# iden3/snarkjs

Hardware: AMD Instinct MI355X
Metric: groth16_proofs_per_sec (higher is better)
Workload: dtype u32; 1 GPU; BN254 Groth16 prove, 2^20 constraints, synthetic zkey/wtns (BASELINE configs[1]), B density 1.0 (every section dense, SURVEY 8d recipe), uniform witness; key + witness resident in HBM; curve=bn128, log_n=20, n_vars=1048571, n_coef=2097203, witness=uniform, coef_dist=flat, parallelism=replica x1 (one proof stream per GPU, 2 proof(s) in flight)

## Files before the change

### snarkjs_amd/csrc/msm29.cuh

```cuda
#pragma once
#include "field29.cuh"
#include "msm.cuh"

namespace zkmi {

#if defined(ZK29_SHADOW)
}
#include <map>
namespace zkmi {
namespace b29 {
struct Parked { double bv, bl, bt; };
inline std::map<const void*, Parked>& parked() { static std::map<const void*, Parked> m; return m; }
}
#endif
template <class C> struct Aff29 { Fp29<C> x, y; };
template <class C> struct XYZZ29 { Fp29<C> X, Y, ZZ, ZZZ; };

template <class C> ZK_HD void dbl_affine29(XYZZ29<C>& r, const Aff29<C>& q) {
    Fp29<C> U = add29(q.y, q.y); norm29(U);
    const Fp29<C> V = mul29(U, U), W = mul29(U, V), S = mul29(q.x, V), xx = mul29(q.x, q.x);
    Fp29<C> M = add29(add29(xx, xx), xx); norm29(M);
    Fp29<C> X3 = sub29<C, 2>(sub29<C, 2>(mul29(M, M), S), S); norm29(X3);
    const Fp29<C> T = sub29<C, 6>(S, X3);
    Fp29<C> Y3 = sub29<C, 2>(mul29(M, T), mul29(W, q.y)); norm29(Y3);
    r.X = X3; r.Y = Y3; r.ZZ = V; r.ZZZ = W;
}
template <class C> ZK_HD void madd29(XYZZ29<C>& acc, bool& inf, const Aff29<C>& q) {
    if (inf) { acc.X = q.x; acc.Y = q.y; acc.ZZ = one29<C>(); acc.ZZZ = one29<C>(); inf = false; return; }
    const Fp29<C> U2 = mul29(q.x, acc.ZZ), S2 = mul29(q.y, acc.ZZZ);
    Fp29<C> P = sub29<C, 8>(U2, acc.X); norm29(P);
    Fp29<C> R = sub29<C, 4>(S2, acc.Y); norm29(R);
    if (is_zero29(P)) {
        if (is_zero29(R)) dbl_affine29(acc, q); else inf = true;
        return;
    }
    const Fp29<C> PP = sqr29(P);
    const Fp29<C> PPP = mul29(P, PP), Q = mul29(acc.X, PP);
    Fp29<C> X3 = sub29<C, 2>(sub29<C, 2>(sub29<C, 2>(sqr29(R), PPP), Q), Q); norm29(X3);
    Fp29<C> T = sub29<C, 8>(Q, X3); norm29(T);
    const Fp29<C> Y3 = mul29_2(R, T, sub29<C, 4>(zero29<C>(), acc.Y), PPP);
    acc.ZZ = mul29(acc.ZZ, PP); acc.ZZZ = mul29(acc.ZZZ, PPP);
    acc.X = X3; acc.Y = Y3;
}
template <class C, bool KEEP29 = false> ZK_HD void store_xyzz29(uint32_t* dst, const XYZZ29<C>& a, bool inf) {
    constexpr int N = C::N;
    if (inf) {
#pragma unroll
        for (int i = 0; i < N; i++) reinterpret_cast<uint4*>(dst)[i] = make_uint4(0, 0, 0, 0);
        return;
    }
    store_r256<C, KEEP29>(dst, a.X); store_r256<C, KEEP29>(dst + N, a.Y); store_r256<C, KEEP29>(dst + 2 * N, a.ZZ); store_r256<C, KEEP29>(dst + 3 * N, a.ZZZ);
}
template <class C> ZK_HD bool load_xyzz29(XYZZ29<C>& a, const uint32_t* src) {
    constexpr int N = C::N;
    const uint4* q = reinterpret_cast<const uint4*>(src + 2 * N);
    uint32_t nz = 0;
#pragma unroll
    for (int i = 0; i < N / 4; i++) { const uint4 z = q[i]; nz |= z.x | z.y | z.z | z.w; }
    if (!nz) return false;
    a.X = load29_packed<C>(src); a.Y = load29_packed<C>(src + N); a.ZZ = load29_packed<C>(src + 2 * N); a.ZZZ = load29_packed<C>(src + 3 * N);
    return true;
}
template <class C> ZK_HD void dbl_xyzz29(XYZZ29<C>& r) {
    Fp29<C> U = add29(r.Y, r.Y); norm29(U);
    const Fp29<C> V = sqr29(U), W = mul29(U, V), S = mul29(r.X, V), xx = sqr29(r.X);
    Fp29<C> M = add29(add29(xx, xx), xx); norm29(M);
    Fp29<C> X3 = sub29<C, 2>(sub29<C, 2>(sqr29(M), S), S); norm29(X3);
    Fp29<C> T = sub29<C, 6>(S, X3); norm29(T);
    const Fp29<C> Y3 = mul29_2(M, T, sub29<C, 2>(zero29<C>(), W), r.Y);
    r.ZZ = mul29(V, r.ZZ); r.ZZZ = mul29(W, r.ZZZ);
    r.X = X3; r.Y = Y3;
}
template <class C, class Ld> ZK_HD void padd29_ld(XYZZ29<C>& acc, bool& inf, Ld ld) {
    if (inf) { acc.X = ld(0); acc.Y = ld(1); acc.ZZ = ld(2); acc.ZZZ = ld(3); inf = false; return; }
    const Fp29<C> U1 = mul29(acc.X, ld(2)), U2 = mul29(ld(0), acc.ZZ);
    Fp29<C> P = sub29<C, 2>(U2, U1); norm29(P);
    const Fp29<C> S1 = mul29(acc.Y, ld(3)), S2 = mul29(ld(1), acc.ZZZ);
    Fp29<C> R = sub29<C, 2>(S2, S1); norm29(R);
    if (is_zero29(P)) {
        if (is_zero29(R)) dbl_xyzz29(acc); else inf = true;
        return;
    }
    const Fp29<C> PP = sqr29(P);
    const Fp29<C> PPP = mul29(P, PP), Q = mul29(U1, PP);
    Fp29<C> X3 = sub29<C, 2>(sub29<C, 2>(sub29<C, 2>(sqr29(R), PPP), Q), Q); norm29(X3);
    Fp29<C> T = sub29<C, 8>(Q, X3); norm29(T);
    const Fp29<C> Y3 = mul29_2(R, T, sub29<C, 2>(zero29<C>(), S1), PPP);
    acc.ZZ = mul29(mul29(acc.ZZ, ld(2)), PP); acc.ZZZ = mul29(mul29(acc.ZZZ, ld(3)), PPP);
    acc.X = X3; acc.Y = Y3;
}
template <class C> ZK_HD void padd29(XYZZ29<C>& acc, bool& inf, const XYZZ29<C>& p) {
    padd29_ld(acc, inf, [&](int k) -> Fp29<C> { return k == 0 ? p.X : (k == 1 ? p.Y : (k == 2 ? p.ZZ : p.ZZZ)); });
}
template <class C> ZK_HD bool xyzz29_words_inf(const uint32_t* src) {
    const uint4* q = reinterpret_cast<const uint4*>(src + 2 * C::N);
    uint32_t nz = 0;
#pragma unroll
    for (int i = 0; i < C::N / 4; i++) { const uint4 z = q[i]; nz |= z.x | z.y | z.z | z.w; }
    return nz == 0;
}


template <class C> ZK_HD bool xyzz29_words_inf_g2(const uint32_t* src) {
    const uint4* q = reinterpret_cast<const uint4*>(src + 4 * C::N);
    uint32_t nz = 0;
#pragma unroll
    for (int i = 0; i < C::N / 2; i++) { const uint4 z = q[i]; nz |= z.x | z.y | z.z | z.w; }
    return nz == 0;
}

template <class C> __global__ void __launch_bounds__(256) k_table_to_r29(uint32_t* __restrict__ table, size_t n_elems) {
    const size_t i = (size_t)blockIdx.x * blockDim.x + threadIdx.x;
    if (i >= n_elems) return;
    Fp<C> v = fp_load<C>(table + i * C::N);
#pragma unroll
    for (int k = 0; k < r29_shift<C>(); k++) v = fp_dbl(v);
    fp_store<C>(table + i * C::N, v);
}

struct ListReader {
    const uint4* sorted4;
    uint32_t a, a_end, at = 0xffffffffu;
    uint4 buf;
    ZK_DEV ListReader(const uint32_t* sorted, uint32_t first, uint32_t last) : sorted4(reinterpret_cast<const uint4*>(sorted)), a(first), a_end(last), buf(make_uint4(0, 0, 0, 0)) {}
    ZK_DEV bool more() const { return a < a_end; }
    ZK_DEV uint32_t next() {
        const uint32_t grp = a >> 2, sel = a & 3u;
        if (grp != at) { buf = sorted4[grp]; at = grp; }
        a++;
        return sel == 0 ? buf.x : (sel == 1 ? buf.y : (sel == 2 ? buf.z : buf.w));
    }
};
#ifndef ZK_SPEC_GATHER
#define ZK_SPEC_GATHER 1
#endif
#ifndef ZK_SPEC_GATHER_G2
#define ZK_SPEC_GATHER_G2(C) (ZK_SPEC_GATHER && Lim29<C>::NL > 9)
#endif
struct SpecEntry { uint32_t e, m, s; };
ZK_DEV bool spec_dead(const SpecEntry& x) { return x.s >= 32u || ((x.m >> x.s) & 1u); }
template <class C> ZK_DEV Fp29<C> unpack29_v(const uint4* v) {
    uint32_t w[C::N];
#pragma unroll
    for (int i = 0; i < C::N / 4; i++) { w[4 * i] = v[i].x; w[4 * i + 1] = v[i].y; w[4 * i + 2] = v[i].z; w[4 * i + 3] = v[i].w; }
    return unpack29<C>(w);
}

template <class C, bool MERGE> __global__ void __launch_bounds__(256, 2)
k_msm_accum29(const uint32_t* __restrict__ bases, const uint32_t* __restrict__ infmask, MsmShape sh, uint32_t skip, uint32_t cap, const uint32_t* __restrict__ counts,
              const uint32_t* __restrict__ starts, const uint32_t* __restrict__ sorted, const uint32_t* __restrict__ lane_g, const uint32_t* __restrict__ lane_sub,
              const uint32_t* __restrict__ meta, uint32_t* __restrict__ buckets, uint32_t* __restrict__ lane_partials, const uint32_t* __restrict__ prev_counts, int bucket_r29) {
    constexpr int N = C::N, PW = 4 * N, AV = N / 2;
    const uint32_t lane = blockIdx.x * blockDim.x + threadIdx.x;
    if (lane >= meta[0]) return;
    const uint32_t g = lane_g[lane];
    const uint32_t cnt = counts[g];
    const uint32_t j = msm_key_lanes_log(msm_key(cnt, cap), cap);
    uint32_t lo = 0, hi = cnt;
    if (j) {
        const uint32_t chunk = (cnt + (1u << j) - 1) >> j;
        lo = min(cnt, lane_sub[lane] * chunk);
        hi = min(cnt, lo + chunk);
    }
    XYZZ29<C> acc;
    bool inf = true;
    if (MERGE) {
        if (prev_counts[g] && (!j || lane_sub[lane] == 0)) {
            const uint32_t* b = buckets + (size_t)g * PW;
            if (bucket_r29) inf = !load_xyzz29(acc, b);
            else {
                uint32_t nz = 0;
#pragma unroll
                for (int i = 0; i < N / 4; i++) { const uint4 z = reinterpret_cast<const uint4*>(b + 2 * N)[i]; nz |= z.x | z.y | z.z | z.w; }
                if (nz) { acc.X = from_r256<C>(b); acc.Y = from_r256<C>(b + N); acc.ZZ = from_r256<C>(b + 2 * N); acc.ZZZ = from_r256<C>(b + 3 * N); inf = false; }
            }
        }
    }
    const uint32_t s0 = starts[g];
    ListReader list(sorted, s0 + lo, s0 + hi);
    struct Raw { uint4 v[AV]; };
    auto fetch = [&](uint32_t& e_out, Raw& r_out) -> bool {
        while (list.more()) {
            const uint32_t e = list.next();
            uint32_t idx = e & 0x7fffffffu;
            if (idx < skip) continue;
            idx -= skip;
            if ((infmask[idx >> 5] >> (idx & 31)) & 1u) continue;
            const uint4* p = reinterpret_cast<const uint4*>(bases + (size_t)idx * (2 * N));
#pragma unroll
            for (int i = 0; i < AV; i++) r_out.v[i] = p[i];
            e_out = e;
            return true;
        }
        return false;
    };
#if ZK_SPEC_GATHER
    auto fetch_spec = [&](SpecEntry& x, Raw& r_out) -> bool {
        if (!list.more()) return false;
        const uint32_t e = list.next();
        uint32_t idx = e & 0x7fffffffu;
        const bool mine = idx >= skip;
        idx = mine ? idx - skip : 0u;
        x.e = e; x.s = mine ? (idx & 31u) : 32u;
        x.m = infmask[idx >> 5];
        const uint4* p = reinterpret_cast<const uint4*>(bases + (size_t)idx * (2 * N));
#pragma unroll
        for (int i = 0; i < AV; i++) r_out.v[i] = p[i];
        return true;
    };
    SpecEntry x_next{0, 0, 32};
    Raw r_next;
    bool have = fetch_spec(x_next, r_next);
    while (have) {
        SpecEntry x = x_next;
        Raw r = r_next;
        have = fetch_spec(x_next, r_next);
        while (spec_dead(x) && have) { x = x_next; r = r_next; have = fetch_spec(x_next, r_next); }
        if (spec_dead(x)) break;
        Aff29<C> q;
        q.x = unpack29_v<C>(r.v); q.y = unpack29_v<C>(r.v + AV / 2);
        if (x.e >> 31) { q.y = sub29<C, 2>(zero29<C>(), q.y); norm29(q.y); }
        madd29(acc, inf, q);
    }
#else
    uint32_t e_next = 0;
    Raw r_next;
    bool have = fetch(e_next, r_next);
    while (have) {
        const uint32_t e = e_next;
        const Raw r = r_next;
        have = fetch(e_next, r_next);
        Aff29<C> q;
        q.x = unpack29_v<C>(r.v); q.y = unpack29_v<C>(r.v + AV / 2);
        if (e >> 31) { q.y = sub29<C, 2>(zero29<C>(), q.y); norm29(q.y); }
        madd29(acc, inf, q);
    }
#endif
    if (j) store_xyzz29<C, false>(lane_partials + (size_t)lane * PW, acc, inf);
    else if (bucket_r29) store_xyzz29<C, true>(buckets + (size_t)g * PW, acc, inf);
    else store_xyzz29<C, false>(buckets + (size_t)g * PW, acc, inf);
}

template <class C> __global__ void __launch_bounds__(256, Lim29<C>::NL <= 9 ? 3 : 2)
k_msm_rowcol_wave29(MsmReduceBatch rb, uint32_t W, uint32_t nb, uint32_t rbits, uint32_t cbits, uint32_t* __restrict__ out) {
    constexpr int NL = Lim29<C>::NL, PW = 4 * C::N;
    extern __shared__ __attribute__((aligned(16))) uint32_t lds[];
    __shared__ uint32_t inf_s[256];
    const uint32_t Cn = 1u << cbits, R = 1u << rbits;
    const uint32_t t = threadIdx.x, sub = t & 63u;
    const size_t n_out = (size_t)rb.njobs * W * 2 * Cn;
    for (size_t blk = blockIdx.x; blk * 4 < n_out; blk += gridDim.x) {
        const size_t gw = blk * 4 + (t >> 6);
        const bool valid = gw < n_out;
        const uint32_t i = (uint32_t)(gw & (Cn - 1)), kind = (uint32_t)(gw >> cbits) & 1u;
        const size_t jw = gw >> (cbits + 1);
        const uint32_t w = (uint32_t)(jw % W), job = (uint32_t)(jw / W);
        XYZZ29<C> acc;
        bool inf = true;
        if (valid) {
            const uint32_t* bk = rb.buckets[job];
            const uint32_t* cn = rb.counts[job];
            const uint32_t cnt = kind ? R : Cn;
            if (!kind && i >= R) {  }
            else for (uint32_t e = sub; e < cnt; e += 64) {
                const size_t g = (size_t)w * nb + (kind ? ((size_t)e << cbits) + i : ((size_t)i << cbits) + e);
                const uint32_t* src = bk + g * PW;
                if (cn[g] && !xyzz29_words_inf<C>(src)) padd29_ld(acc, inf, [&](int k) { return load29_packed<C>(src + k * C::N); });
            }
        }
        uint32_t* mine = lds + t;
        for (uint32_t d = 1; d < 64; d <<= 1) {
            inf_s[t] = inf ? 1u : 0u;
            if (!inf) {
#pragma unroll
                for (int k = 0; k < NL; k++) { mine[k * 256] = acc.X.l[k]; mine[(NL + k) * 256] = acc.Y.l[k]; mine[(2 * NL + k) * 256] = acc.ZZ.l[k]; mine[(3 * NL + k) * 256] = acc.ZZZ.l[k]; }
            }
            __syncthreads();
            if ((t & (2 * d - 1)) == 0 && !inf_s[t + d]) {
                const uint32_t* pn = lds + t + d;
                padd29_ld(acc, inf, [&](int k) { Fp29<C> v;
#pragma unroll
                    for (int i = 0; i < NL; i++) v.l[i] = pn[(k * NL + i) * 256];
                    return v; });
            }
            __syncthreads();
        }
        if (valid && sub == 0) store_xyzz29<C, false>(out + gw * PW, acc, inf);
    }
}

template <class C> struct F2x { Fp29<C> c0, c1; };
template <class C, int K> ZK_HD Fp29<C> neg29(const Fp29<C>& a) { Fp29<C> r = sub29<C, K>(zero29<C>(), a); norm29(r); return r; }
#define ZK_F2_CALLS(C) (IsCompact<C>::value)
template <class C> __host__ __device__ ZK_NOINLINE_DEV F2x<C> f2mul_call(F2x<C> a, F2x<C> b) {
    static_assert(Lim29<C>::NL > 9, "called Fq2 product: 14-limb curve only (offset 16 p needs its headroom)");
    const Fp29<C> nb1 = neg29<C, 16>(b.c1);
    return F2x<C>{mul29_2_inl(a.c0, b.c0, a.c1, nb1), mul29_2_inl(a.c0, b.c1, a.c1, b.c0)};
}
template <class C> ZK_HD F2x<C> f2mul(const F2x<C>& a, const F2x<C>& b, const Fp29<C>& nb1) {
    if constexpr (ZK_F2_CALLS(C)) return f2mul_call<C>(a, b);
    else return F2x<C>{mul29_2(a.c0, b.c0, a.c1, nb1), mul29_2(a.c0, b.c1, a.c1, b.c0)};
}
template <class C, int KB> ZK_HD F2x<C> f2sqr(const F2x<C>& a) {
    Fp29<C> s = add29(a.c0, a.c1), d = sub29<C, KB>(a.c0, a.c1);
    norm29(d);
    Fp29<C> t = mul29(a.c0, a.c1);
    Fp29<C> c1 = add29(t, t);
    norm29(c1);
    return F2x<C>{mul29(s, d), c1};
}
template <class C, int K> ZK_HD F2x<C> f2sub(const F2x<C>& a, const F2x<C>& b) { return F2x<C>{sub29<C, K>(a.c0, b.c0), sub29<C, K>(a.c1, b.c1)}; }
template <class C> ZK_HD void f2norm(F2x<C>& a) { norm29(a.c0); norm29(a.c1); }
template <class C> ZK_HD bool f2zero(const F2x<C>& a) { return is_zero29(a.c0) && is_zero29(a.c1); }

template <class C, int T, bool PACK> struct LdsAcc29 {
    static constexpr int NL = Lim29<C>::NL, EW = PACK ? C::N : NL;
    uint32_t* base;
    ZK_HD void get1(int slot, Fp29<C>& v) const {
        if constexpr (PACK) {
            uint32_t w[C::N];
#pragma unroll
            for (int i = 0; i < C::N; i++) w[i] = base[(slot * EW + i) * T];
            v = unpack29<C>(w);
        } else {
#pragma unroll
            for (int i = 0; i < NL; i++) v.l[i] = base[(slot * EW + i) * T];
        }
#if defined(ZK29_SHADOW)
        {
            auto it = b29::parked().find(&base[(size_t)slot * EW * T]);
            b29::need(it != b29::parked().end(), "LdsAcc29: slot read before it was written", slot, 0);
            if (it != b29::parked().end()) { v.bv = it->second.bv; v.bl = it->second.bl; v.bt = it->second.bt; }
        }
#endif
    }
    ZK_HD void put1(int slot, const Fp29<C>& v) const {
#if defined(ZK29_SHADOW)
        {
            b29::need(b29::normalised(v), "LdsAcc29: a parked value is not normalised", v.bl, b29::lowmax<C>());
            b29::Parked pk; pk.bv = v.bv; pk.bl = v.bl; pk.bt = v.bt;
            b29::parked()[&base[(size_t)slot * EW * T]] = pk;
        }
#endif
        if constexpr (PACK) {
            uint32_t w[C::N];
            pack29<C>(w, v);
#pragma unroll
            for (int i = 0; i < C::N; i++) base[(slot * EW + i) * T] = w[i];
        } else {
#pragma unroll
            for (int i = 0; i < NL; i++) base[(slot * EW + i) * T] = v.l[i];
        }
    }
    ZK_HD void get(int coord, F2x<C>& v) const { get1(2 * coord, v.c0); get1(2 * coord + 1, v.c1); }
    ZK_HD void put(int coord, const F2x<C>& v) const { put1(2 * coord, v.c0); put1(2 * coord + 1, v.c1); }
};
#ifndef ZK_Y3_SPLIT
#define ZK_Y3_SPLIT(C) (Lim29<C>::NL > 9 || IsCompact<C>::value)
#endif
#ifndef ZK_G2_PREFETCH
#define ZK_G2_PREFETCH(C) true
#endif
#if defined(__HIP_DEVICE_COMPILE__)
#define ZK_SFENCE() __builtin_amdgcn_sched_barrier(0)
#else
#define ZK_SFENCE() ((void)0)
#endif
template <class C, class Acc> ZK_HD void madd29_lds(const Acc& A, bool& inf, const F2x<C>& qx, const F2x<C>& qy) {
    F2x<C> t;
    if (inf) {
        A.put(0, qx); A.put(1, qy);
        t.c0 = one29<C>(); t.c1 = zero29<C>();
        A.put(2, t); A.put(3, t);
        inf = false;
        return;
    }
    A.get(2, t);
    const F2x<C> U2 = f2mul(t, qx, neg29<C, 2>(qx.c1));
    ZK_SFENCE();
    A.get(0, t);
    F2x<C> P = f2sub<C, 9>(U2, t); f2norm(P);
    A.get(3, t);
    const F2x<C> S2 = f2mul(t, qy, neg29<C, 3>(qy.c1));
    ZK_SFENCE();
    A.get(1, t);
    F2x<C> R = f2sub<C, 4>(S2, t); f2norm(R);
    if (f2zero(P)) {
        if (f2zero(R)) {
            F2x<C> U{add29(qy.c0, qy.c0), add29(qy.c1, qy.c1)}; f2norm(U);
            const F2x<C> V = f2sqr<C, 5>(U);
            const Fp29<C> nV1 = neg29<C, 3>(V.c1);
            const F2x<C> W = f2mul(U, V, nV1), S = f2mul(qx, V, nV1);
            const F2x<C> xx = f2sqr<C, 2>(qx);
            F2x<C> M{add29(add29(xx.c0, xx.c0), xx.c0), add29(add29(xx.c1, xx.c1), xx.c1)}; f2norm(M);
            F2x<C> X3 = f2sub<C, 2>(f2sub<C, 2>(f2sqr<C, 7>(M), S), S); f2norm(X3);
            F2x<C> Tt = f2sub<C, 7>(S, X3); f2norm(Tt);
            const F2x<C> MT = f2mul(M, Tt, neg29<C, 9>(Tt.c1)), Wy = f2mul(W, qy, neg29<C, 3>(qy.c1));
            F2x<C> Y3 = f2sub<C, 2>(MT, Wy); f2norm(Y3);
            A.put(0, X3); A.put(1, Y3); A.put(2, V); A.put(3, W);
        } else inf = true;
        return;
    }
    const F2x<C> PP = f2sqr<C, 11>(P);
    ZK_SFENCE();
    const Fp29<C> nPP1 = neg29<C, 4>(PP.c1);
    const F2x<C> PPP = f2mul(P, PP, nPP1);
    ZK_SFENCE();
    const Fp29<C> nPPP1 = neg29<C, 2>(PPP.c1);
    A.get(2, t); A.put(2, f2mul(t, PP, nPP1));
    ZK_SFENCE();
    A.get(3, t); A.put(3, f2mul(t, PPP, nPPP1));
    ZK_SFENCE();
    A.get(0, t);
    const F2x<C> Q = f2mul(t, PP, nPP1);
    ZK_SFENCE();
    F2x<C> X3 = f2sub<C, 2>(f2sub<C, 2>(f2sub<C, 2>(f2sqr<C, 6>(R), PPP), Q), Q); f2norm(X3);
    A.put(0, X3);
    ZK_SFENCE();
    F2x<C> Tq = f2sub<C, 9>(Q, X3); f2norm(Tq);
    const Fp29<C> nR1 = neg29<C, 6>(R.c1);
    F2x<C> Y3;
    if constexpr (ZK_Y3_SPLIT(C)) {
        const F2x<C> TR{mul29_2(Tq.c0, R.c0, Tq.c1, nR1), mul29_2(Tq.c0, R.c1, Tq.c1, R.c0)};
        ZK_SFENCE();
        const Fp29<C> nPPP0 = neg29<C, 2>(PPP.c0);
        A.get(1, t);
        Y3.c0 = add29(TR.c0, mul29_2(t.c0, nPPP0, t.c1, PPP.c1));
        Y3.c1 = add29(TR.c1, mul29_2(t.c0, nPPP1, t.c1, nPPP0));
        f2norm(Y3);
    } else {
        const Fp29<C> nPPP0 = neg29<C, 2>(PPP.c0);
        A.get(1, t);
        Y3.c0 = mul29_4(Tq.c0, R.c0, Tq.c1, nR1, t.c0, nPPP0, t.c1, PPP.c1);
        Y3.c1 = mul29_4(Tq.c0, R.c1, Tq.c1, R.c0, t.c0, nPPP1, t.c1, nPPP0);
    }
    A.put(1, Y3);
}
template <class C, class Acc, bool KEEP29 = false> ZK_HD void store_xyzz29_lds(uint32_t* dst, const Acc& A, bool inf) {
    constexpr int N = C::N;
    if (inf) {
#pragma unroll
        for (int i = 0; i < 2 * N; i++) reinterpret_cast<uint4*>(dst)[i] = make_uint4(0, 0, 0, 0);
// ... 496 lines not shown
```

### snarkjs_amd/csrc/msm_host.hpp

```cpp
#pragma once
#include <stdlib.h>
#include <string.h>
#include <algorithm>
#include "host_field.hpp"
#include "msm.cuh"
#include "msm29.cuh"
#include <type_traits>
#include "zkmi_common.hpp"
#include "msm_select.hpp"

namespace zkmi {

static inline int ilog2_sz(size_t n) { int l = 0; while (((size_t)1 << (l + 1)) <= n) l++; return l; }

static inline int msm_pick_c(size_t n) {
    int lg = ilog2_sz(n ? n : 1);
    if (lg < 62 && n > (((size_t)3) << lg) / 2) lg++;
    static const int T[] = {2, 2, 2, 3, 3, 4, 4, 5, 6, 7, 8, 9, 9, 10, 11, 11, 12, 15, 15, 15, 15, 15, 16, 16, 16, 16, 16, 16, 16, 16, 16, 16};
    return T[lg > 31 ? 31 : lg];
}

template <class F> struct HostOf;
template <> struct HostOf<Fp<Bn254Fq>> { typedef host::HField<4> FT; static FT make() { return host::HField<4>::from_cfg<Bn254Fq>(); } };
template <> struct HostOf<Fp2<Bn254Fq>> { typedef host::HField2<4> FT; static FT make() { return FT{host::HField<4>::from_cfg<Bn254Fq>()}; } };
// ... 46 lines not shown
template <class F> int to_affine_host(const uint8_t* jac, uint8_t* aff) {
    typedef typename HostOf<F>::FT FT;
    host::HCurve<FT> cv{HostOf<F>::make()};
    constexpr int FW = FieldWords<F>::value;
    typename host::HCurve<FT>::P p;
    memcpy(&p.X, jac, 4 * FW); memcpy(&p.Y, jac + 4 * FW, 4 * FW); memcpy(&p.Z, jac + 8 * FW, 4 * FW);
    typename FT::E x, y;
    cv.to_affine(p, x, y);
    memcpy(aff, &x, 4 * FW); memcpy(aff + 4 * FW, &y, 4 * FW);
    return ZKMI_OK;
}

struct MsmPlan {
    MsmShape sh;
    int slot = 0;
    size_t total = 0;
    uint32_t cap = 0;
    size_t lane_bound = 0, multi_bound = 0;
    uint32_t *counts = nullptr, *starts = nullptr, *sorted = nullptr;
    uint32_t *lane_g = nullptr, *lane_sub = nullptr, *meta = nullptr, *giants = nullptr;
    struct Path {
        int nw = 0;
        bool radix = false, staged = false;
        uint32_t lb = 0, parts = 0, fused_cap = 0;
        const uint32_t* chunk_meta = nullptr;
    } path;
};
constexpr int MSM_TB = 128, MSM_LOG_TB = 7;
int msm_sort(const void* d_scalars, size_t n, size_t sb, MsmPlan& plan, int plan_slot = 0, int precomp_c = 0, size_t table_stride = 0, const uint32_t* d_dropmask = nullptr);

struct MsmJob {
    int W = 0, c = 0, cbits = 0, slot = 0;
    bool merged = false;
    bool r29 = false;
    int bitsums = 0;
    uint32_t nb = 0;
    uint32_t* h_win = nullptr;
    const uint32_t *buckets = nullptr, *counts = nullptr;
    hipEvent_t acc0 = nullptr, acc1 = nullptr;
};
constexpr int MSM_JOB_SLOTS = 8;
constexpr size_t MSM_JOB_SLOT_BYTES = 512 * 1024;
int msm_job_slot(int slot, MsmJob& job);

template <auto Kernel> int lds_opt_in(size_t bytes) {
    static bool opted = false;
    if (!opted) {
        ZK_HIP(hipFuncSetAttribute((const void*)Kernel, hipFuncAttributeMaxDynamicSharedMemorySize, (int)bytes));
        opted = true;
    }
    return ZKMI_OK;
}
static inline int msm_pick_fail(MsmPickError e) { return fail(msm_pick_code(e), msm_pick_message(e)); }

template <class F> int msm_accumulate(const void* d_bases, const MsmPlan& pl, uint32_t skip, MsmJob& job, const uint32_t* d_infmask = nullptr, MsmJob* into = nullptr) {
    constexpr int FW = FieldWords<F>::value, PW = 4 * FW;
    constexpr bool WIDE = FW > 12;
    typedef typename F::Cfg C;
    constexpr int NL = Lim29<C>::NL;
    static_assert(!WIDE || (Accum29G2<C>::T == msm_wide_block(NL) && MsmAccumBlock<F>::value == msm_wide_block(NL)), "msm_select.hpp: block of the Fq2 kernels");
    static_assert(G2S_SLOTS == MSM_G2S_LANES, "msm_select.hpp: lanes per block of k_msm_accum29_g2s");
    Ctx& cx = ctx();
    const MsmShape& sh = pl.sh;
    const size_t total = pl.total;
    hipStream_t st = cx.stream;
    const std::string sfx = "." + std::to_string(job.slot);
    auto r29 = cx.r29_tables.find(d_bases);
    const bool table29 = r29 != cx.r29_tables.end();
    const int box = table29 && (WIDE || NL > 9) ? compact_code() : 0;
    const MsmAccumPick pick = msm_accum_pick(WIDE ? 2 : 1, NL, table29, into != nullptr, into && into->r29, sh.c, box, msm_tuning());
    if (pick.error == MsmPickError::merge_g2) return msm_pick_fail(pick.error);
    uint32_t *buckets, *lane_partials, *block_partials;
    const uint32_t* prev_counts = nullptr;
    if (into) {
        if (into->W != sh.W || into->c != sh.c || into->nb != sh.nb || !into->buckets) return fail(ZKMI_ERR_INVALID, "msm_accumulate: merge target of a different shape");
        buckets = const_cast<uint32_t*>(into->buckets);
        prev_counts = into->counts;
    } else ZK_TRY(ws_get("msm.buckets" + sfx, total * PW * 4, (void**)&buckets));
    if (pick.error != MsmPickError::none) return msm_pick_fail(pick.error);
    ZK_TRY(ws_get("msm.lane_partials", std::max<size_t>(pl.multi_bound, 1) * PW * 4, (void**)&lane_partials));
    const size_t tree_blocks = pl.multi_bound / MSM_TB + 1;
    ZK_TRY(ws_get("msm.block_partials", tree_blocks * PW * 4, (void**)&block_partials));
    const size_t tree_lds = (size_t)MSM_TB * PW * 4;
    ZK_TRY((lds_opt_in<k_msm_tree<F, MSM_TB>>(tree_lds)));
    ZK_TRY((lds_opt_in<k_msm_giant<F, MSM_TB>>(tree_lds)));
    const dim3 grid((unsigned)((pl.lane_bound + pick.lanes_per_block - 1) / pick.lanes_per_block)), block(pick.threads);
    const uint32_t* mask = d_infmask ? d_infmask : (table29 ? r29->second : nullptr);
    const int r29_flag = (int)pick.r29_buckets;
    auto launch29 = [&](auto kernel) {
        hipLaunchKernelGGL(kernel, grid, block, 0, st, (const uint32_t*)d_bases, mask, sh, skip, pl.cap, pl.counts, pl.starts, pl.sorted, pl.lane_g, pl.lane_sub, pl.meta, buckets,
                           lane_partials, prev_counts, r29_flag);
    };
    auto launch29_g2 = [&](auto kernel, size_t lds) {
        hipLaunchKernelGGL(kernel, grid, block, lds, st, (const uint32_t*)d_bases, mask, sh, skip, pl.cap, pl.counts, pl.starts, pl.sorted, pl.lane_g, pl.lane_sub, pl.meta, buckets,
                           lane_partials, r29_flag);
    };
    auto launch32 = [&](auto kernel, size_t lds) {
        hipLaunchKernelGGL(kernel, grid, block, lds, st, (const uint32_t*)d_bases, mask, sh, skip, pl.cap, pl.counts, pl.starts, pl.sorted, pl.lane_g, pl.lane_sub, pl.meta, buckets,
                           lane_partials, prev_counts);
    };
    if (job.acc0) ZK_HIP(hipEventRecord(job.acc0, st));
    typedef MsmAccumKernel K;
    switch (pick.kernel) {
    case K::accum29: if constexpr (!WIDE) launch29(k_msm_accum29<C, false>); break;
    case K::accum29_merge: if constexpr (!WIDE) launch29(k_msm_accum29<C, true>); break;
    case K::accum29_compact: if constexpr (!WIDE && NL > 9) launch29(k_msm_accum29<Compact<C>, false>); break;
    case K::accum29_compact_merge: if constexpr (!WIDE && NL > 9) launch29(k_msm_accum29<Compact<C>, true>); break;
    case K::accum29_g2s: if constexpr (WIDE) launch29_g2(k_msm_accum29_g2s<C>, 0); break;
    case K::accum29_g2:
    case K::accum29_g2_compact:
        if constexpr (WIDE) {
            constexpr size_t lds29 = Accum29G2<C>::lds_bytes;
            ZK_TRY(lds_opt_in<k_msm_accum29_g2<C>>(lds29));
            if constexpr (NL > 9) {
                ZK_TRY(lds_opt_in<k_msm_accum29_g2<Compact<C>>>(lds29));
                if (pick.kernel == K::accum29_g2_compact) { launch29_g2(k_msm_accum29_g2<Compact<C>>, lds29); break; }
            }
            launch29_g2(k_msm_accum29_g2<C>, lds29);
        }
        break;
    case K::accum32: if constexpr (!WIDE) launch32(k_msm_accum<F, false, false>, 0); break;
    case K::accum32_merge: if constexpr (!WIDE) launch32(k_msm_accum<F, false, true>, 0); break;
    case K::accum32_wide:
        if constexpr (WIDE) {
            const size_t acc_lds = (size_t)PW * pick.threads * 4;
            ZK_TRY((lds_opt_in<k_msm_accum<F, true, false>>(acc_lds)));
            launch32(k_msm_accum<F, true, false>, acc_lds);
        }
        break;
    }
    if (job.acc1) ZK_HIP(hipEventRecord(job.acc1, st));
    if (cx.msm_stats && cx.d_addcount && job.slot < MSM_JOB_SLOTS) {
        const int ci = cx.pipe * MSM_JOB_SLOTS + job.slot;
        ZK_HIP(hipMemsetAsync(cx.d_addcount + ci, 0, 8, st));
        hipLaunchKernelGGL(k_msm_count_adds, dim3(1024), dim3(256), 0, st, pl.sorted, pl.counts, pl.starts, (uint32_t)total, skip, mask, cx.d_addcount + ci);
        ZK_HIP(hipMemcpyAsync(cx.h_addcount + ci, cx.d_addcount + ci, 8, hipMemcpyDeviceToHost, st));
    }
    hipLaunchKernelGGL((k_msm_tree<F, MSM_TB>), dim3((unsigned)std::min<size_t>(tree_blocks, 512)), dim3(MSM_TB), tree_lds, st, lane_partials, pl.lane_g, pl.counts, pl.cap, pl.meta, buckets,
                       block_partials, r29_flag);
    hipLaunchKernelGGL((k_msm_giant<F, MSM_TB>), dim3((unsigned)std::min<size_t>(tree_blocks, 256)), dim3(MSM_TB), tree_lds, st, pl.giants, pl.meta, block_partials, buckets, r29_flag);
    job.W = sh.W; job.c = sh.c; job.nb = sh.nb; job.buckets = buckets; job.counts = pl.counts;
    job.merged = into != nullptr;
    job.r29 = pick.r29_buckets;
    if (into) {
        uint32_t* cmb;
        ZK_TRY(ws_get("msm.cmbcounts." + std::to_string(into->slot), total * 4, (void**)&cmb));
        hipLaunchKernelGGL(k_msm_counts_add, dim3((unsigned)((total + 255) / 256)), dim3(256), 0, st, prev_counts, pl.counts, (uint32_t)total, cmb);
        into->counts = cmb;
    }
    ZK_HIP(hipGetLastError());
    return ZKMI_OK;
}

template <class F> int msm_reduce(MsmJob* const* jobs, int njobs, bool aux = false) {
    constexpr int FW = FieldWords<F>::value, PW = 4 * FW;
    Ctx& cx = ctx();
    hipStream_t st = aux ? cx.aux_stream : cx.stream;
    const std::string ax = aux ? ".aux" : "";
    if (njobs < 1 || njobs > MSM_MAX_BATCH) return fail(ZKMI_ERR_INVALID, "msm_reduce: bad batch size");
    const int W = jobs[0]->W, c = jobs[0]->c;
    const uint32_t nb = jobs[0]->nb;
    MsmReduceBatch rb;
    rb.njobs = njobs;
    for (int i = 0; i < njobs; i++) {
        if (jobs[i]->W != W || jobs[i]->c != c) return fail(ZKMI_ERR_INVALID, "msm_reduce: jobs of different shape");
        rb.buckets[i] = jobs[i]->buckets; rb.counts[i] = jobs[i]->counts;
    }
    const uint32_t rbits = (uint32_t)(c - 1) / 2, cbits = (uint32_t)(c - 1) - rbits, C = 1u << cbits;
    const size_t VW = (size_t)njobs * W * 2;
    constexpr int M = (PW * 4 * 2 * 256 <= 128 * 1024) ? 256 : 128;
    const uint32_t m2 = (C + M - 1) / M;
    uint32_t *rc, *a0, *r0, *a1, *r1;
    ZK_TRY(ws_get("msm.rowcol" + ax, VW * C * PW * 4, (void**)&rc));
    ZK_TRY(ws_get("msm.redA0" + ax, std::max<size_t>(VW * m2, VW * (cbits + 1)) * PW * 4, (void**)&a0));
    ZK_TRY(ws_get("msm.redR0" + ax, VW * m2 * PW * 4, (void**)&r0));
    ZK_TRY(ws_get("msm.redA1" + ax, VW * PW * 4, (void**)&a1));
    ZK_TRY(ws_get("msm.redR1" + ax, VW * PW * 4, (void**)&r1));
    const size_t n_out = VW * C;
    constexpr bool WIDE_R = FW > 12;
    typedef typename F::Cfg Cfg;
    constexpr int NL = Lim29<Cfg>::NL;
    static_assert(MsmRcBlock<F>::value == (WIDE_R ? msm_wide_block(NL) : 256u) && (!WIDE_R || Reduce29G2<Cfg>::T == msm_wide_block(NL)), "msm_select.hpp: block of the wave sums");
    bool all_r29 = true;
    for (int i = 0; i < njobs; i++) all_r29 = all_r29 && jobs[i]->r29;
    for (int i = 0; i < njobs; i++) if (jobs[i]->r29 != jobs[0]->r29) return fail(ZKMI_ERR_INVALID, "msm_reduce: jobs with different bucket formats");
    const int box = !WIDE_R && NL > 9 && all_r29 ? compact_code() : 0;
    const MsmRowcolPick rp = msm_rowcol_pick(WIDE_R ? 2 : 1, NL, all_r29, rbits, cbits, aux, box, msm_tuning());
    if (rp.error != MsmPickError::none) return msm_pick_fail(rp.error);
    const size_t per_block = rp.threads / 64, rc_blocks = std::min((n_out + per_block - 1) / per_block, rp.max_blocks);
    auto launch_wave = [&](auto kernel, size_t lds) {
        hipLaunchKernelGGL(kernel, dim3((unsigned)rc_blocks), dim3(rp.threads), lds, st, rb, (uint32_t)W, nb, rbits, cbits, rc);
    };
    switch (rp.kernel) {
    case MsmRowcolKernel::wave29:
    case MsmRowcolKernel::wave29_compact:
        if constexpr (!WIDE_R) {
            constexpr size_t lds29 = (size_t)256 * 4 * NL * 4;
            ZK_TRY(lds_opt_in<k_msm_rowcol_wave29<Cfg>>(lds29));
            if constexpr (NL > 9) {
                ZK_TRY(lds_opt_in<k_msm_rowcol_wave29<Compact<Cfg>>>(lds29));
                if (rp.kernel == MsmRowcolKernel::wave29_compact) { launch_wave(k_msm_rowcol_wave29<Compact<Cfg>>, lds29); break; }
            }
            launch_wave(k_msm_rowcol_wave29<Cfg>, lds29);
        }
        break;
    case MsmRowcolKernel::wave29_g2:
        if constexpr (WIDE_R) {
            ZK_TRY(lds_opt_in<k_msm_rowcol_wave29_g2<Cfg>>(Reduce29G2<Cfg>::lds_bytes));
            launch_wave(k_msm_rowcol_wave29_g2<Cfg>, Reduce29G2<Cfg>::lds_bytes);
        }
        break;
    case MsmRowcolKernel::wave: {
        const size_t lds_rc = (size_t)rp.threads * PW * 4;
        ZK_TRY(lds_opt_in<k_msm_rowcol_wave<F>>(lds_rc));
        launch_wave(k_msm_rowcol_wave<F>, lds_rc);
        break;
    }
    case MsmRowcolKernel::staged: {
        const uint32_t seq = WIDE_R ? 4 : 16, maxL = WIDE_R ? 256 : 64, foldK = WIDE_R ? 4 : 8;
        uint32_t L = 1;
        while (L < maxL && (C / L) > seq) L <<= 1;
        uint32_t *p0, *p1;
        ZK_TRY(ws_get("msm.rcpart0" + ax, n_out * L * PW * 4, (void**)&p0));
        ZK_TRY(ws_get("msm.rcpart1" + ax, std::max<size_t>(n_out * L / 4, 1) * PW * 4, (void**)&p1));
        uint32_t* dst = L == 1 ? rc : p0;
        hipLaunchKernelGGL((k_msm_rowcol<F>), dim3((unsigned)((n_out * L + 255) / 256)), dim3(256), 0, st, rb, (uint32_t)W, nb, rbits, cbits, L, dst);
        uint32_t parts = L;
        const uint32_t* src = dst;
        while (parts > 1) {
            const uint32_t K = std::min<uint32_t>(parts, foldK);
            parts /= K;
            uint32_t* d2 = parts == 1 ? rc : (src == p0 ? p1 : p0);
            hipLaunchKernelGGL((k_msm_fold<F>), dim3((unsigned)((n_out * parts + 255) / 256)), dim3(256), 0, st, src, d2, n_out * parts, K);
            src = d2;
        }
        break;
    }
    }
    const bool bitsums = VW * (cbits + 1) <= 256;
    const uint32_t* resA = nullptr;
    const uint32_t* resR = nullptr;
    size_t perA = 0;
    if (bitsums) {
        const dim3 bgrid((unsigned)(VW * (cbits + 1)));
        if (rp.bitsums_lds) {
            if constexpr (WIDE_R) {
                constexpr int TB = MsmAccumBlock<F>::value;
                ZK_TRY(lds_opt_in<k_msm_bitsums_lds<F>>((size_t)TB * PW * 4));
                hipLaunchKernelGGL((k_msm_bitsums_lds<F>), bgrid, dim3(TB), (size_t)TB * PW * 4, st, rc, C, cbits, a0);
            }
        } else {
            constexpr int MB = (PW * 4 * 256 <= 64 * 1024) ? 256 : 128;
            ZK_TRY((lds_opt_in<k_msm_bitsums<F, MB>>((size_t)MB * PW * 4)));
            hipLaunchKernelGGL((k_msm_bitsums<F, MB>), bgrid, dim3(MB), (size_t)MB * PW * 4, st, rc, C, cbits, a0);
        }
        resA = a0;
        perA = (size_t)2 * W * (cbits + 1) * PW;
    } else {
        uint32_t m = C;
        int log_scale = 0;
        const uint32_t *inA = nullptr, *inR = rc;
        uint32_t *outA = a0, *outR = r0;
        const size_t lds_ws = (size_t)2 * M * PW * 4;
        ZK_TRY((lds_opt_in<k_msm_wsum<F, M>>(lds_ws)));
        for (;;) {
            const uint32_t blocks = (m + M - 1) / M;
            hipLaunchKernelGGL((k_msm_wsum<F, M>), dim3((unsigned)(VW * blocks)), dim3(M), lds_ws, st, inA, inR, m, blocks, log_scale, outA, outR);
            inA = outA; inR = outR;
            if (blocks == 1) break;
            outA = (outA == a0) ? a1 : a0; outR = (outR == r0) ? r1 : r0;
            m = blocks;
            log_scale += ilog2_sz(M);
        }
        resA = inA; resR = inR;
        perA = (size_t)2 * W * PW;
    }
    for (int i = 0; i < njobs; i++) {
        MsmJob& job = *jobs[i];
        job.cbits = (int)cbits;
        job.bitsums = bitsums ? 1 : 0;
        if (perA * 4 * 2 > MSM_JOB_SLOT_BYTES) return fail(ZKMI_ERR_UNSUPPORTED, "msm: too many windows");
        ZK_HIP(hipMemcpyAsync(job.h_win, resA + (size_t)i * perA, perA * 4, hipMemcpyDeviceToHost, st));
        if (!bitsums) ZK_HIP(hipMemcpyAsync(job.h_win + perA, resR + (size_t)i * perA, perA * 4, hipMemcpyDeviceToHost, st));
    }
    ZK_HIP(hipGetLastError());
    return ZKMI_OK;
}
template <class F> void msm_fold(const MsmJob& job, uint8_t* out_jac) {
    constexpr int PW = 4 * FieldWords<F>::value;
    if (job.merged) { memset(out_jac, 0, 3 * PW); return; }
    if (!job.bitsums) { msm_fold_windows<F>(job.h_win, job.h_win + (size_t)2 * job.W * PW, job.W, job.c, job.cbits, out_jac); return; }
    typedef typename HostOf<F>::FT FT;
    host::HCurve<FT> cv{HostOf<F>::make()};
    const int nb1 = job.cbits + 1;
    std::vector<uint32_t> win((size_t)2 * job.W * PW), tot((size_t)2 * job.W * PW);
    auto put = [&](uint32_t* dst, const typename host::HCurve<FT>::P& p) {
        constexpr int FW = FieldWords<F>::value;
        if (cv.is_zero(p)) { memset(dst, 0, PW * 4); return; }
        auto z2 = cv.F.sqr(p.Z), z3 = cv.F.mul(z2, p.Z);
        memcpy(dst, &p.X, 4 * FW); memcpy(dst + FW, &p.Y, 4 * FW); memcpy(dst + 2 * FW, &z2, 4 * FW); memcpy(dst + 3 * FW, &z3, 4 * FW);
    };
    for (int a = 0; a < 2 * job.W; a++) {
        const uint32_t* src = job.h_win + (size_t)a * nb1 * PW;
        auto acc = cv.zero();
        for (int k = job.cbits - 1; k >= 0; k--) { if (!cv.is_zero(acc)) acc = cv.dbl(acc); acc = cv.add(acc, xyzz_to_jac<F>(cv, src + (size_t)k * PW)); }
        put(win.data() + (size_t)a * PW, acc);
        memcpy(tot.data() + (size_t)a * PW, src + (size_t)job.cbits * PW, PW * 4);
    }
    msm_fold_windows<F>(win.data(), tot.data(), job.W, job.c, job.cbits, out_jac);
}

template <class F> int msm_run(const void* d_bases, const void* d_scalars, size_t n, size_t sb, uint8_t* out_jac) {
    constexpr int FW = FieldWords<F>::value;
    Ctx& cx = ctx();
    if (n == 0) { memset(out_jac, 0, 3 * 4 * FW); return ZKMI_OK; }
    hipStream_t st = cx.stream;
    MsmPlan pl;
    MsmJob job;
    ZK_TRY(slot_idle_or_fail("msm"));
    ZK_TRY(msm_job_slot(0, job));
    if (!cx.ev0_held) ZK_HIP(hipEventRecord(cx.ev0, st));
    ZK_TRY(msm_sort(d_scalars, n, sb, pl));
    ZK_TRY(msm_accumulate<F>(d_bases, pl, 0, job));
    MsmJob* jp = &job;
    ZK_TRY(msm_reduce<F>(&jp, 1));
    ZK_HIP(hipEventRecord(cx.ev1, st));
    ZK_HIP(hipStreamSynchronize(st));
    float ms = 0;
    if (hipEventElapsedTime(&ms, cx.ev0, cx.ev1) == hipSuccess) cx.last_ms = ms;
    msm_fold<F>(job, out_jac);
    return ZKMI_OK;
}

static inline int msm_precomp_c(size_t n) {
    int lg = ilog2_sz(n ? n : 1);
    if (lg < 62 && n > (((size_t)3) << lg) / 2) lg++;
    int c = std::max(8, std::min(21, lg));
    if (lg >= 14) { static const int snap[] = {15, 15, 16, 17, 17, 20, 20, 20}; c = snap[std::min(std::max(c, 14), 21) - 14]; }
    return c;
}
static inline int msm_digits(size_t sb, int c) { return (int)((8 * sb + 1 + c - 1) / c); }
template <class F> int msm_precompute(const void* d_bases, size_t n, int c, int Wd, void* d_table) {
    Ctx& cx = ctx();
    hipLaunchKernelGGL((k_msm_precompute<F>), dim3((unsigned)((n + 255) / 256)), dim3(256), 0, cx.stream, (const uint32_t*)d_bases, (uint32_t)n, c, Wd, (uint32_t*)d_table);
    ZK_HIP(hipGetLastError());
    return ZKMI_OK;
}
int msm_precompute_dispatch(int curve, int group, const void* d_bases, size_t n, int c, int Wd, void* d_table);
template <class F> int msm_infmask(const void* d_points, size_t n, uint32_t* d_mask) {
    Ctx& cx = ctx();
    ZK_HIP(hipMemsetAsync(d_mask, 0, ((n + 31) / 32) * 4, cx.stream));
    if (n) hipLaunchKernelGGL((k_msm_infmask<F>), dim3((unsigned)((n + 255) / 256)), dim3(256), 0, cx.stream, (const uint32_t*)d_points, n, d_mask);
    ZK_HIP(hipGetLastError());
    return ZKMI_OK;
}
template <class F> int msm_run_table(const void* d_table, size_t stride, int c, const void* d_scalars, size_t k, size_t sb, uint8_t* out_jac);
// ... 137 lines not shown
```

Before: 113.0 proofs/s.

## Plan row/column bucket sums with variable lane counts and cross-wave LDS folds

Replaces the fixed one-wave-per-sum row/column reduction kernel with a planned task list. Each sum now gets 64 to 256 lanes, chosen by a host-side planner that balances total adds against the longest chain and against the chip's wave slots. Partial sums are folded through LDS in a pairwise tree across waves, and the longer kind is scheduled first. The cost is extra __syncthreads and LDS traffic for the cross-wave fold, plus a more complex indexing path.

Measured after the change: 112.7 proofs/s. No clear change (-0.3%).

```diff
diff --git a/snarkjs_amd/csrc/msm29.cuh b/snarkjs_amd/csrc/msm29.cuh
--- a/snarkjs_amd/csrc/msm29.cuh
+++ b/snarkjs_amd/csrc/msm29.cuh
@@ -1,6 +1,7 @@
 #pragma once
 #include "field29.cuh"
 #include "msm.cuh"
+#include "msm_rowcol_plan.hpp"
 
 namespace zkmi {
 
@@ -241,6 +242,91 @@
     else store_xyzz29<C, false>(buckets + (size_t)g * PW, acc, inf);
 }
 
+#ifndef ZK_ROWCOL_COMPACT_FOLD
+#define ZK_ROWCOL_COMPACT_FOLD 1
+#endif
+template <class C, int T> ZK_HD void park_xyzz29(uint32_t* lds, uint32_t s, const XYZZ29<C>& a) {
+    constexpr int NL = Lim29<C>::NL;
+    uint32_t* m = lds + s;
+#pragma unroll
+    for (int k = 0; k < NL; k++) { m[k * T] = a.X.l[k]; m[(NL + k) * T] = a.Y.l[k]; m[(2 * NL + k) * T] = a.ZZ.l[k]; m[(3 * NL + k) * T] = a.ZZZ.l[k]; }
+}
+template <class C, int T> ZK_HD Fp29<C> parked29(const uint32_t* lds, uint32_t s, int k) {
+    constexpr int NL = Lim29<C>::NL;
+    Fp29<C> v;
+#pragma unroll
+    for (int i = 0; i < NL; i++) v.l[i] = lds[(k * NL + i) * T + s];
+    return v;
+}
+template <class C, int T> ZK_HD void unpark_xyzz29(XYZZ29<C>& a, const uint32_t* lds, uint32_t s) {
+    a.X = parked29<C, T>(lds, s, 0); a.Y = parked29<C, T>(lds, s, 1); a.ZZ = parked29<C, T>(lds, s, 2); a.ZZZ = parked29<C, T>(lds, s, 3);
+}
+template <class C, int T> ZK_HD void rowcol_step29(XYZZ29<C>& acc, bool& inf, bool fold, bool work, const uint32_t* src, uint32_t* lds, uint32_t* inf_s, uint32_t a, uint32_t b) {
+    if (fold) {
+        work = work && !inf_s[b];
+        if (work) { inf = inf_s[a] != 0; if (!inf) unpark_xyzz29<C, T>(acc, lds, a); }
+    }
+    else if (work) {
+        XYZZ29<C> p;
+        p.X = load29_packed<C>(src); p.Y = load29_packed<C>(src + C::N); p.ZZ = load29_packed<C>(src + 2 * C::N); p.ZZZ = load29_packed<C>(src + 3 * C::N);
+        park_xyzz29<C, T>(lds, b, p);
+    }
+    if (work) padd29_ld(acc, inf, [&](int k) { return parked29<C, T>(lds, b, k); });
+    if (fold && work) {
+        inf_s[a] = inf ? 1u : 0u;
+        if (!inf) park_xyzz29<C, T>(lds, a, acc);
+    }
+}
+#if ZK_ROWCOL_COMPACT_FOLD
+template <class C> __global__ void __launch_bounds__(256, Lim29<C>::NL <= 9 ? 3 : 2)
+k_msm_rowcol_wave29(MsmReduceBatch rb, uint32_t W, uint32_t nb, uint32_t rbits, uint32_t cbits, MsmRowcolPlan plan, uint32_t* __restrict__ out) {
+    constexpr int PW = 4 * C::N, T = 256;
+    extern __shared__ __attribute__((aligned(16))) uint32_t lds[];
+    __shared__ uint32_t inf_s[T];
+    const uint32_t Cn = 1u << cbits, R = 1u << rbits, t = threadIdx.x;
+    for (uint32_t b = blockIdx.x; b < plan.n_tasks; b += gridDim.x) {
+        const MsmRowcolTask tk = msm_rowcol_task(plan, rbits, cbits, b);
+        const uint32_t lanes_log = plan.lanes_log[tk.kind], share = tk.len >> lanes_log;
+        const uint32_t i = tk.first_sum + (t >> lanes_log), sub = t & (tk.lanes - 1u);
+        const uint32_t w = tk.jw % W, job = tk.jw / W;
+        const uint32_t* bk = rb.buckets[job];
+        const uint32_t* cn = rb.counts[job];
+        XYZZ29<C> acc;
+        bool inf = true;
+#pragma unroll 1
+        for (uint32_t step = 0; step < share + lanes_log; step++) {
+            const bool fold = step >= share;
+            const uint32_t* src = bk;
+            uint32_t sa = t, sb = t;
+            bool work;
+            if (!fold) {
+                const size_t g = (size_t)w * nb + msm_rowcol_bucket(tk.kind, cbits, i, sub + (step << lanes_log));
+                src = bk + g * PW;
+                work = cn[g] && !xyzz29_words_inf<C>(src);
+            } else {
+                const uint32_t d = 1u << (step - share);
+                if (step == share) {
+                    inf_s[t] = inf ? 1u : 0u;
+                    if (!inf) park_xyzz29<C, T>(lds, t, acc);
+                }
+                __syncthreads();
+                work = t < msm_fold_pairs(T, d);
+                sa = work ? msm_fold_acc_slot(d, t) : t; sb = work ? msm_fold_op_slot(d, t) : t;
+            }
+            rowcol_step29<C, T>(acc, inf, fold, work, src, lds, inf_s, sa, sb);
+        }
+        __syncthreads();
+        if (sub == 0) {
+            uint32_t* dst = out + (((size_t)tk.jw * 2 + tk.kind) * Cn + i) * PW;
+            inf = inf_s[t] != 0;
+            if (!inf) unpark_xyzz29<C, T>(acc, lds, t);
+            store_xyzz29<C, false>(dst, acc, inf);
+            if (!tk.kind && R < Cn) store_xyzz29<C, false>(dst + (size_t)R * PW, acc, true);
+        }
+        __syncthreads();
+    }
+}
+#else
 template <class C> __global__ void __launch_bounds__(256, Lim29<C>::NL <= 9 ? 3 : 2)
 k_msm_rowcol_wave29(MsmReduceBatch rb, uint32_t W, uint32_t nb, uint32_t rbits, uint32_t cbits, uint32_t* __restrict__ out) {
     constexpr int NL = Lim29<C>::NL, PW = 4 * C::N;
@@ -288,6 +374,7 @@
         if (valid && sub == 0) store_xyzz29<C, false>(out + gw * PW, acc, inf);
     }
 }
+#endif
 
 template <class C> struct F2x { Fp29<C> c0, c1; };
 template <class C, int K> ZK_HD Fp29<C> neg29(const Fp29<C>& a) { Fp29<C> r = sub29<C, K>(zero29<C>(), a); norm29(r); return r; }
diff --git a/snarkjs_amd/csrc/msm_host.hpp b/snarkjs_amd/csrc/msm_host.hpp
--- a/snarkjs_amd/csrc/msm_host.hpp
+++ b/snarkjs_amd/csrc/msm_host.hpp
@@ -222,6 +222,15 @@
     return ZKMI_OK;
 }
 
+inline uint64_t chip_wave_slots(int waves_per_simd) {
+    static const int cus = [] {
+        int dev = 0, n = 0;
+        if (hipGetDevice(&dev) != hipSuccess || hipDeviceGetAttribute(&n, hipDeviceAttributeMultiprocessorCount, dev) != hipSuccess || n <= 0) { (void)hipGetLastError(); n = 256; }
+        return n;
+    }();
+    return (uint64_t)cus * 4 * waves_per_simd;
+}
+
 template <class F> int msm_reduce(MsmJob* const* jobs, int njobs, bool aux = false) {
     constexpr int FW = FieldWords<F>::value, PW = 4 * FW;
     Ctx& cx = ctx();
@@ -266,12 +275,21 @@
     case MsmRowcolKernel::wave29_compact:
         if constexpr (!WIDE_R) {
             constexpr size_t lds29 = (size_t)256 * 4 * NL * 4;
+#if ZK_ROWCOL_COMPACT_FOLD
+            const uint64_t slots = rp.max_blocks != SIZE_MAX ? (uint64_t)rp.max_blocks * per_block : chip_wave_slots(NL <= 9 ? 3 : 2);
+            const MsmRowcolPlan plan = msm_rowcol_plan((uint32_t)njobs, (uint32_t)W, rbits, cbits, rp.threads, slots);
+            auto launch_plan = [&](auto kernel, size_t lds) {
+                hipLaunchKernelGGL(kernel, dim3((unsigned)std::min<size_t>(plan.n_tasks, rp.max_blocks)), dim3(rp.threads), lds, st, rb, (uint32_t)W, nb, rbits, cbits, plan, rc);
+            };
+#else
+            auto launch_plan = launch_wave;
+#endif
             ZK_TRY(lds_opt_in<k_msm_rowcol_wave29<Cfg>>(lds29));
             if constexpr (NL > 9) {
                 ZK_TRY(lds_opt_in<k_msm_rowcol_wave29<Compact<Cfg>>>(lds29));
-                if (rp.kernel == MsmRowcolKernel::wave29_compact) { launch_wave(k_msm_rowcol_wave29<Compact<Cfg>>, lds29); break; }
+                if (rp.kernel == MsmRowcolKernel::wave29_compact) { launch_plan(k_msm_rowcol_wave29<Compact<Cfg>>, lds29); break; }
             }
-            launch_wave(k_msm_rowcol_wave29<Cfg>, lds29);
+            launch_plan(k_msm_rowcol_wave29<Cfg>, lds29);
         }
         break;
     case MsmRowcolKernel::wave29_g2:
diff --git a/snarkjs_amd/csrc/msm_rowcol_plan.hpp b/snarkjs_amd/csrc/msm_rowcol_plan.hpp
--- /dev/null
+++ b/snarkjs_amd/csrc/msm_rowcol_plan.hpp
@@ -0,0 +1,86 @@
+#pragma once
+#include <stddef.h>
+#include <stdint.h>
+
+#if defined(__HIPCC__) || defined(__CUDACC__)
+#define ZK_PLAN_HD __host__ __device__ inline
+#else
+#define ZK_PLAN_HD inline
+#endif
+
+namespace zkmi {
+
+ZK_PLAN_HD uint32_t msm_fold_acc_slot(uint32_t d, uint32_t k) { return 2u * d * k; }
+ZK_PLAN_HD uint32_t msm_fold_op_slot(uint32_t d, uint32_t k) { return 2u * d * k + d; }
+ZK_PLAN_HD uint32_t msm_fold_pairs(uint32_t T, uint32_t d) { return T / (2u * d); }
+ZK_PLAN_HD uint32_t msm_fold_wave_adds(uint32_t T, uint32_t L) {
+    uint32_t n = 0;
+    for (uint32_t d = 1; d < L; d <<= 1) n += (msm_fold_pairs(T, d) + 63u) / 64u;
+    return n;
+}
+
+struct MsmRowcolPlan {
+    uint32_t lanes_log[2];
+    uint32_t blocks[2];
+    uint32_t first_kind;
+    uint32_t n_first;
+    uint32_t n_tasks;
+    uint32_t threads;
+    uint64_t wave_adds;
+};
+struct MsmRowcolTask {
+    uint32_t kind, jw, first_sum, sums, lanes, len;
+};
+ZK_PLAN_HD MsmRowcolTask msm_rowcol_task(const MsmRowcolPlan& p, uint32_t rbits, uint32_t cbits, uint32_t b) {
+    MsmRowcolTask t;
+    t.kind = b < p.n_first ? p.first_kind : 1u - p.first_kind;
+    const uint32_t bb = b < p.n_first ? b : b - p.n_first;
+    t.jw = bb / p.blocks[t.kind];
+    t.lanes = 1u << p.lanes_log[t.kind];
+    t.sums = p.threads >> p.lanes_log[t.kind];
+    t.first_sum = (bb % p.blocks[t.kind]) * t.sums;
+    t.len = 1u << (t.kind ? rbits : cbits);
+    return t;
+}
+ZK_PLAN_HD size_t msm_rowcol_bucket(uint32_t kind, uint32_t cbits, uint32_t i, uint32_t e) {
+    return kind ? ((size_t)e << cbits) + i : ((size_t)i << cbits) + e;
+}
+
+inline uint64_t msm_rowcol_wave_adds(uint32_t jobs, uint32_t W, uint32_t rbits, uint32_t cbits, uint32_t T, uint32_t rl, uint32_t cl) {
+    const uint64_t R = 1ull << rbits, Cn = 1ull << cbits, wpb = T / 64;
+    const uint64_t row_blocks = R / (T >> rl), col_blocks = Cn / (T >> cl);
+    return (uint64_t)jobs * W * (row_blocks * (wpb * (Cn >> rl) + msm_fold_wave_adds(T, 1u << rl)) + col_blocks * (wpb * (R >> cl) + msm_fold_wave_adds(T, 1u << cl)));
+}
+inline uint64_t msm_rowcol_wave_adds_tree(uint32_t jobs, uint32_t W, uint32_t rbits, uint32_t cbits) {
+    const uint64_t R = 1ull << rbits, Cn = 1ull << cbits;
+    return (uint64_t)jobs * W * (R * (Cn / 64 + 6) + Cn * (R / 64 + 6));
+}
+
+inline MsmRowcolPlan msm_rowcol_plan(uint32_t jobs, uint32_t W, uint32_t rbits, uint32_t cbits, uint32_t T, uint64_t wave_slots) {
+    const uint64_t R = 1ull << rbits, Cn = 1ull << cbits, JW = (uint64_t)jobs * W;
+    const bool underfill = JW * (R + Cn) <= wave_slots;
+    uint32_t best_rl = 6, best_cl = 6;
+    uint64_t best_key[3] = {~0ull, ~0ull, ~0ull};
+    for (uint32_t rl = 6; rl <= 8 && (1u << rl) <= T && rl <= cbits; rl++)
+        for (uint32_t cl = 6; cl <= 8 && (1u << cl) <= T && cl <= rbits; cl++) {
+            const uint64_t waves = JW * ((R << rl) + (Cn << cl)) / 64, adds = msm_rowcol_wave_adds(jobs, W, rbits, cbits, T, rl, cl);
+            if (underfill && waves > wave_slots) continue;
+            const uint64_t rs = Cn >> rl, cs = R >> cl;
+            const uint64_t chain = (rs + rl > cs + cl) ? rs + rl : cs + cl;
+            const uint64_t key[3] = {underfill ? chain : adds, underfill ? adds : (rs > cs ? rs - cs : cs - rs), (uint64_t)rl + cl};
+            bool better = false;
+            for (int i = 0; i < 3; i++) if (key[i] != best_key[i]) { better = key[i] < best_key[i]; break; }
+            if (better) { best_rl = rl; best_cl = cl; for (int i = 0; i < 3; i++) best_key[i] = key[i]; }
+        }
+    MsmRowcolPlan p;
+    p.lanes_log[0] = best_rl; p.lanes_log[1] = best_cl;
+    p.blocks[0] = (uint32_t)(R / (T >> best_rl)); p.blocks[1] = (uint32_t)(Cn / (T >> best_cl));
+    p.first_kind = (Cn >> best_rl) >= (R >> best_cl) ? 0u : 1u;
+    p.n_first = (uint32_t)(JW * p.blocks[p.first_kind]);
+    p.n_tasks = (uint32_t)(JW * (p.blocks[0] + p.blocks[1]));
+    p.threads = T;
+    p.wave_adds = msm_rowcol_wave_adds(jobs, W, rbits, cbits, T, best_rl, best_cl);
+    return p;
+}
+
+}
```
